# dotnetpower/infomesh

Hardware: AMD Instinct MI355X
Metric: queries/sec (hybrid BM25+dense search, 1.25M docs) (higher is better)
Workload: dtype bf16; 1 GPU; model=bge-small-en(random-init) encoder + BM25 CSR + cosine top-k, global_batch=128, seq_len=32, parallelism=shard1, mode=hybrid, docs_per_gpu=1250000, total_docs=1250000

## Files before the change

### infomesh_amd/models/bert.py

```python
from __future__ import annotations

from dataclasses import dataclass

import torch

from ..ops import kernels as K
from ..ops import reference as R


@dataclass(frozen=True)
class BertConfig:
    vocab_size: int
    hidden: int
    layers: int
    heads: int
    ffn: int
    max_pos: int = 512
    eps: float = 1e-12

    @property
    def head_dim(self) -> int:
        return self.hidden // self.heads


# ... 32 lines not shown
        t = v.to(device)
        out[k] = t if k.endswith(".b") and "ln" not in k else t.to(dtype)
        if "ln" in k:
            out[k] = t.to(dtype)
    return out


class BertEncoder:
    def __init__(self, cfg: BertConfig, weights: dict[str, torch.Tensor],
                 use_fused_attn: bool = True):
        self.cfg = cfg
        self.w = weights
        self.use_fused_attn = use_fused_attn and cfg.head_dim in (32, 64,
                                                                  96, 128)

    def forward(self, ids: torch.Tensor, lens: torch.Tensor) -> torch.Tensor:
        cfg, w = self.cfg, self.w
        B, S = ids.shape
        if S % 32 != 0:
            pad = 32 - S % 32
            ids = torch.nn.functional.pad(ids, (0, pad))
            S += pad
        H, nh, d = cfg.hidden, cfg.heads, cfg.head_dim
        pos_ids = torch.arange(S, device=ids.device, dtype=torch.int32)\
            .repeat(B)
        x = K.gather(w["embed.word"], ids.reshape(-1))
        x = K.add(x, K.gather(w["embed.pos"], pos_ids))
        x = K.layernorm(x, w["embed.ln.g"], w["embed.ln.b"], eps=cfg.eps)

        vl = lens.repeat_interleave(nh).contiguous()
        scale = d ** -0.5
        vl_b = lens.contiguous()
        for i in range(cfg.layers):
            p = f"layer.{i}."
            qkv = K.gemm_nt(x, w[p + "qkv.w"], bias=w[p + "qkv.b"])
            if self.use_fused_attn:
                qkv5 = qkv.view(B, S, 3, nh, d)
                qv = qkv5[:, :, 0].permute(0, 2, 1, 3)
                kv = qkv5[:, :, 1].permute(0, 2, 1, 3)
                vv = qkv5[:, :, 2].permute(0, 2, 1, 3)
                ctx = K.attn_fused(qv, kv, vv, valid_len=vl_b, scale=scale)
            else:
                q, k, vt = K.qkv_split(qkv, B, S, nh, nh, d)
                scores = K.gemm_nt(q, k, out_f32=True, alpha=scale)
                probs = K.softmax(scores, valid_len=vl)
                ctx = K.gemm_nt(probs, vt)
            merged = K.merge_heads(ctx, B, S, nh, d)
            attn = K.gemm_nt(merged, w[p + "attn_out.w"],
                             bias=w[p + "attn_out.b"])
            x = K.layernorm(attn, w[p + "ln1.g"], w[p + "ln1.b"],
                            residual=x, eps=cfg.eps)
            h = K.gemm_nt(x, w[p + "ffn_in.w"], bias=w[p + "ffn_in.b"],
                          act="gelu")
            o = K.gemm_nt(h, w[p + "ffn_out.w"], bias=w[p + "ffn_out.b"])
            x = K.layernorm(o, w[p + "ln2.g"], w[p + "ln2.b"],
                            residual=x, eps=cfg.eps)
        return x.view(B, S, H)

    def forward_reference(self, ids: torch.Tensor,
                          lens: torch.Tensor) -> torch.Tensor:
        cfg = self.cfg
        w = {k: v.float().cpu() for k, v in self.w.items()}
        B, S = ids.shape
        H, nh, d = cfg.hidden, cfg.heads, cfg.head_dim
        ids_l = ids.cpu().long()
        x = w["embed.word"][ids_l] + w["embed.pos"][:S].unsqueeze(0)
        x = R.layernorm(x, w["embed.ln.g"], w["embed.ln.b"], eps=cfg.eps)
        vl = lens.cpu().repeat_interleave(nh)
        for i in range(cfg.layers):
            p = f"layer.{i}."
            qkv = R.gemm_nt(x.view(B * S, H), w[p + "qkv.w"], w[p + "qkv.b"])
            qkv = qkv.view(B, S, 3, nh, d)
# ... 16 lines not shown
```

### infomesh_amd/models/encoder.py

```python
from __future__ import annotations

import torch

from ..ops import kernels as K
from ..ops import reference as R
from .bert import BertConfig, BertEncoder, init_bert_weights
from .tokenizer import HashTokenizer

BGE_SMALL = BertConfig(vocab_size=30522, hidden=384, layers=12, heads=12,
                       ffn=1536, max_pos=512)

EMBED_DIM = BGE_SMALL.hidden


class EmbeddingEncoder:

    def __init__(self, device: str = "cuda", seed: int = 1234,
                 cfg: BertConfig = BGE_SMALL, max_len: int = 128,
                 use_graph: bool = True):
        self.cfg = cfg
        self.device = device
        self.max_len = max_len
        self.tokenizer = HashTokenizer(cfg.vocab_size)
        self.bert = BertEncoder(cfg, init_bert_weights(cfg, seed, device))
        from ..ops.graphs import GraphedCallable
        self._graphed = GraphedCallable(self._encode_impl, enabled=use_graph)

    def _encode_impl(self, ids: torch.Tensor,
                     lens: torch.Tensor) -> torch.Tensor:
        hidden = self.bert.forward(ids, lens)
        return K.pool(hidden, lens, mode="cls", l2=True)

    def encode_ids(self, ids: torch.Tensor, lens: torch.Tensor) -> torch.Tensor:
        return self._graphed(ids, lens)

    def encode_texts(self, texts: list[str]) -> torch.Tensor:
        ids_l, lens = self.tokenizer.encode_batch(texts, self.max_len)
        ids = torch.tensor(ids_l, dtype=torch.int32, device=self.device)
        lens_t = torch.tensor(lens, dtype=torch.int32, device=self.device)
        return self.encode_ids(ids, lens_t)

    def encode_ids_reference(self, ids: torch.Tensor,
                             lens: torch.Tensor) -> torch.Tensor:
        hidden = self.bert.forward_reference(ids, lens)
        return R.pool(hidden.bfloat16(), lens.cpu(), mode="cls", l2=True)
```

### infomesh_amd/models/phi3.py

```python
from __future__ import annotations

from dataclasses import dataclass

import torch

from ..ops import kernels as K
from ..ops import reference as R


@dataclass(frozen=True)
class Phi3Config:
    vocab_size: int = 32064
    hidden: int = 3072
    layers: int = 32
    heads: int = 32
    kv_heads: int = 32
    ffn: int = 8192
    max_pos: int = 4096
    rope_theta: float = 10000.0
    eps: float = 1e-5

    @property
    def head_dim(self) -> int:
        return self.hidden // self.heads
# ... 82 lines not shown
        x = K.gather(self.w["embed"], ids.reshape(-1))
        scale = d ** -0.5
        fused = d in (32, 64, 96, 128)
        for i in range(cfg.layers):
            p = f"layer.{i}."
            h = K.rmsnorm(x, self.w[p + "ln1.g"], eps=cfg.eps)
            qkv = K.gemm_nt(h, self.w[p + "qkv.w"])
            qh, kh, vt = K.qkv_split(qkv, B, S, nh, nkv, d,
                                     cos_t=self.cos, sin_t=self.sin,
                                     pos=pos, want_vt=not fused)
            v_view = qkv.view(B, S, nh + 2 * nkv, d)[:, :, nh + nkv:]\
                .permute(0, 2, 1, 3)
            self.k_cache[i][:B, :, :S] = kh.view(B, nkv, S, d)
            self.v_cache[i][:B, :, :S] = v_view
            if fused:
                ctx = K.attn_fused(qh.view(B, nh, S, d),
                                   kh.view(B, nkv, S, d), v_view,
                                   causal=True, scale=scale)
            else:
                if nh != nkv:
                    rep = nh // nkv
                    kh = kh.view(B, nkv, 1, S, d)\
                        .expand(B, nkv, rep, S, d)\
                        .reshape(B * nh, S, d).contiguous()
                    vt = vt.view(B, nkv, 1, d, S)\
                        .expand(B, nkv, rep, d, S)\
                        .reshape(B * nh, d, S).contiguous()
                scores = K.gemm_nt(qh, kh, out_f32=True, alpha=scale)
                probs = K.softmax(scores, causal=True)
                ctx = K.gemm_nt(probs, vt)
            merged = K.merge_heads(ctx, B, S, nh, d)
            attn = K.gemm_nt(merged, self.w[p + "o.w"])
            x = K.add(x, attn)
            h2 = K.rmsnorm(x, self.w[p + "ln2.g"], eps=cfg.eps)
            gu = K.gemm_nt(h2, self.w[p + "gate_up.w"])
            mlp = K.gemm_nt(K.silu_mul_fused(gu, cfg.ffn),
                            self.w[p + "down.w"])
            x = K.add(x, mlp)
        self.lens[:B] = S_true
        self._len_host = max(self._len_host, S_true)
        x_last = x.view(B, S, H)[:, S_true - 1, :].contiguous()
        h = K.rmsnorm(x_last, self.w["final_ln.g"], eps=cfg.eps)
        return K.gemm_nt(h, self.w["lm_head"], out_f32=True)

    def decode_step(self, ids: torch.Tensor) -> torch.Tensor:
        B = ids.shape[0]
# ... 119 lines not shown
```

### infomesh_amd/models/reranker.py

```python
from __future__ import annotations

import torch

from ..ops import kernels as K
from .bert import BertConfig, BertEncoder, init_bert_weights
from .tokenizer import HashTokenizer, PAD

BGE_RERANKER_BASE = BertConfig(vocab_size=250002, hidden=768, layers=12,
                               heads=12, ffn=3072, max_pos=512)


class CrossEncoderReranker:
    def __init__(self, device: str = "cuda", seed: int = 4321,
                 cfg: BertConfig = BGE_RERANKER_BASE, max_len: int = 160,
                 batch: int = 256):
        self.cfg = cfg
        self.device = device
        self.max_len = max_len
        self.batch = batch
        self.tokenizer = HashTokenizer(cfg.vocab_size)
        self.bert = BertEncoder(cfg, init_bert_weights(cfg, seed, device))
        g = torch.Generator().manual_seed(seed + 1)
        self.cls_w = (torch.randn(1, cfg.hidden, generator=g) * 0.02)\
            .to(device).bfloat16()
        self.cls_b = torch.zeros(1, device=device)

    def score_ids(self, ids: torch.Tensor, lens: torch.Tensor) -> torch.Tensor:
        hidden = self.bert.forward(ids, lens)
        cls = K.pool(hidden, lens, mode="cls", l2=False)
        logits = K.gemm_nt(cls.bfloat16(), self.cls_w, bias=self.cls_b,
                           out_f32=True)
        return logits.view(-1)

    def score_pairs(self, query: str, passages: list[str]) -> torch.Tensor:
        out = []
        for i in range(0, len(passages), self.batch):
            chunk = passages[i:i + self.batch]
            enc = [self.tokenizer.encode_pair(query, p, self.max_len)
                   for p in chunk]
            lens = [len(e) for e in enc]
            width = max(lens)
            ids = torch.tensor([e + [PAD] * (width - len(e)) for e in enc],
                               dtype=torch.int32, device=self.device)
            lens_t = torch.tensor(lens, dtype=torch.int32, device=self.device)
# ... 11 lines not shown
```

### infomesh_amd/ops/_ext.py

```python
from __future__ import annotations

import ctypes
from ctypes import c_float, c_int, c_long, c_void_p
from pathlib import Path

from ..errors import GpuExtensionMissing

_LIB: ctypes.CDLL | None = None
_LOAD_ERROR: str | None = None

_SIGNATURES: dict[str, list] = {
    "infomesh_gemm_bf16_nt": [c_void_p, c_void_p, c_void_p, c_void_p,
                              c_int, c_int, c_int, c_int,
                              c_long, c_long, c_long,
                              c_int, c_float, c_int, c_void_p],
    "infomesh_layernorm": [c_void_p, c_void_p, c_void_p, c_void_p,
                           c_void_p, c_void_p, c_long, c_int, c_float,
                           c_void_p],
    "infomesh_rmsnorm": [c_void_p, c_void_p, c_void_p, c_void_p,
                         c_void_p, c_long, c_int, c_float, c_void_p],
    "infomesh_softmax": [c_void_p, c_void_p, c_void_p, c_long, c_int,
                         c_int, c_int, c_float, c_void_p],
    "infomesh_bias_act": [c_void_p, c_void_p, c_long, c_int, c_int, c_void_p],
    "infomesh_silu_mul": [c_void_p, c_void_p, c_void_p, c_long, c_void_p],
# ... 24 lines not shown
    "infomesh_simhash_fingerprint": [c_void_p, c_void_p, c_void_p, c_long,
                                     c_void_p],
    "infomesh_hamming_scan": [c_void_p, c_void_p, c_void_p, c_void_p,
                              c_void_p, c_void_p, c_int, c_long, c_int,
                              c_int, c_void_p],
    "infomesh_attn_decode": [c_void_p, c_void_p, c_void_p, c_void_p,
                             c_void_p, c_int, c_int, c_int, c_int, c_int,
                             c_float, c_void_p],
    "infomesh_attn_decode_split": [c_void_p, c_void_p, c_void_p, c_void_p,
                                   c_void_p, c_void_p, c_int, c_int, c_int,
                                   c_int, c_int, c_int, c_float, c_void_p],
    "infomesh_attn_fused": [c_void_p, c_void_p, c_void_p, c_void_p,
                            c_void_p, c_int, c_int, c_int, c_int, c_int,
                            c_int, c_long, c_long, c_long, c_long, c_long,
                            c_long, c_long, c_long, c_long,
                            c_int, c_float, c_void_p],
    "infomesh_kv_append": [c_void_p, c_void_p, c_void_p, c_void_p,
                           c_void_p, c_int, c_int, c_int, c_int, c_void_p],
    "infomesh_dense_scores": [c_void_p, c_void_p, c_void_p,
                              c_int, c_long, c_int, c_float, c_void_p],
    "infomesh_dense_scores_fp8": [c_void_p, c_void_p, c_void_p,
                                  c_int, c_long, c_int, c_float,
                                  c_void_p],
    "infomesh_gemm8_bf16_nt": [c_void_p, c_void_p, c_void_p, c_void_p,
                               c_int, c_int, c_int, c_int,
                               c_long, c_long, c_long,
                               c_int, c_float, c_int, c_void_p],
    "infomesh_gemv_bf16_nt": [c_void_p, c_void_p, c_void_p, c_void_p,
                              c_int, c_int, c_int, c_int,
                              c_long, c_long, c_long,
                              c_int, c_float, c_int, c_void_p],
# ... 96 lines not shown
```

### infomesh_amd/ops/csrc/attn_fused.hip

```cpp
#include "common.h"

#define QTILE 64
#define KTILE 64
#define VPAD 72

struct TensorView {
  const bf16* ptr;
  long bs, hs, rs;
};

namespace {

template <int D>
__global__ __launch_bounds__(256) void attn_fused_kernel(
    TensorView Q, TensorView K, TensorView V,
    const int* __restrict__ valid_len,
    bf16* __restrict__ O, int nhq, int nhk,
    int Sq, int Sk, int causal, float scale) {
  __shared__ bf16 k_lds[KTILE][D];
  __shared__ bf16 vt_lds[D][VPAD];
  __shared__ bf16 p_lds[4][16][KTILE];
  const int g = blockIdx.y;
  const int q0 = blockIdx.x * QTILE;
  const int lane = threadIdx.x & 63;
  const int wid = threadIdx.x >> 6;
  const int b = g / nhq, hq = g % nhq;
  const int hk = hq / (nhq / nhk);
  const int limit_all = valid_len ? min(Sk, valid_len[b]) : Sk;

  const bf16* Qg = Q.ptr + (long)b * Q.bs + (long)hq * Q.hs;
  const bf16* Kg = K.ptr + (long)b * K.bs + (long)hk * K.hs;
  const bf16* Vg = V.ptr + (long)b * V.bs + (long)hk * V.hs;

  const int qrow_f = lane & 15;
  const int kslice = lane >> 4;
  bf16x8 qfrag[D / 32];
  {
    const int qr = min(q0 + wid * 16 + qrow_f, Sq - 1);
// ... 2 lines not shown
      qfrag[f] = *reinterpret_cast<const bf16x8*>(
          Qg + (long)qr * Q.rs + f * 32 + kslice * 8);
  }

  f32x4 o_acc[D / 16];
#pragma unroll
  for (int f = 0; f < D / 16; ++f) o_acc[f] = f32x4{0.f, 0.f, 0.f, 0.f};
  float m_run[4], l_run[4];
#pragma unroll
  for (int r = 0; r < 4; ++r) { m_run[r] = -INFINITY; l_run[r] = 0.f; }
  const int crow0 = (lane >> 4) * 4;
  const int ccol = lane & 15;

  int kv_limit = limit_all;
  if (causal) {
    const int max_q = min(q0 + QTILE - 1, Sq - 1);
    kv_limit = min(kv_limit, max_q + (Sk - Sq) + 1);
  }

  for (int kv0 = 0; kv0 < kv_limit; kv0 += KTILE) {
    {
      const int perrow = D / 8;
      for (int t = threadIdx.x; t < KTILE * perrow; t += 256) {
        const int key = t / perrow, dc = (t % perrow) * 8;
        const int src = min(kv0 + key, Sk - 1);
        *reinterpret_cast<bf16x8*>(&k_lds[key][dc]) =
            *reinterpret_cast<const bf16x8*>(Kg + (long)src * K.rs + dc);
        const bf16x8 vv = *reinterpret_cast<const bf16x8*>(
            Vg + (long)src * V.rs + dc);
#pragma unroll
        for (int j = 0; j < 8; ++j) vt_lds[dc + j][key] = vv[j];
      }
    }
    __syncthreads();

    f32x4 s_chunk[KTILE / 16];
#pragma unroll
    for (int kc = 0; kc < KTILE / 16; ++kc) {
      f32x4 acc = f32x4{0.f, 0.f, 0.f, 0.f};
#pragma unroll
      for (int f = 0; f < D / 32; ++f) {
        const bf16x8 kf = *reinterpret_cast<const bf16x8*>(
            &k_lds[kc * 16 + qrow_f][f * 32 + kslice * 8]);
        acc = __builtin_amdgcn_mfma_f32_16x16x32_bf16(
            qfrag[f], kf, acc, 0, 0, 0);
      }
      s_chunk[kc] = acc;
    }

    float tile_max[4];
#pragma unroll
    for (int r = 0; r < 4; ++r) tile_max[r] = -INFINITY;
#pragma unroll
    for (int kc = 0; kc < KTILE / 16; ++kc) {
      const int key = kv0 + kc * 16 + ccol;
      const bool key_ok = key < limit_all;
#pragma unroll
      for (int r = 0; r < 4; ++r) {
        const int qrow = q0 + wid * 16 + crow0 + r;
        bool ok = key_ok && qrow < Sq;
        if (causal) ok = ok && key <= qrow + (Sk - Sq);
        float v = ok ? s_chunk[kc][r] * scale : -INFINITY;
        s_chunk[kc][r] = v;
        tile_max[r] = fmaxf(tile_max[r], v);
      }
    }
#pragma unroll
    for (int r = 0; r < 4; ++r) {
#pragma unroll
      for (int off = 1; off < 16; off <<= 1)
        tile_max[r] = fmaxf(tile_max[r],
                            __shfl_xor(tile_max[r], off, 64));
    }

    float alpha[4];
#pragma unroll
    for (int r = 0; r < 4; ++r) {
      const float m_new = fmaxf(m_run[r], tile_max[r]);
      alpha[r] = (m_run[r] > -INFINITY) ? __expf(m_run[r] - m_new) : 0.f;
      m_run[r] = m_new;
    }
    float row_sum[4] = {0.f, 0.f, 0.f, 0.f};
#pragma unroll
    for (int kc = 0; kc < KTILE / 16; ++kc) {
#pragma unroll
      for (int r = 0; r < 4; ++r) {
        const float p = (s_chunk[kc][r] > -INFINITY && m_run[r] > -INFINITY)
            ? __expf(s_chunk[kc][r] - m_run[r]) : 0.f;
        s_chunk[kc][r] = p;
        row_sum[r] += p;
      }
    }
#pragma unroll
    for (int r = 0; r < 4; ++r) {
#pragma unroll
      for (int off = 1; off < 16; off <<= 1)
        row_sum[r] += __shfl_xor(row_sum[r], off, 64);
      l_run[r] = l_run[r] * alpha[r] + row_sum[r];
    }

#pragma unroll
    for (int f = 0; f < D / 16; ++f)
#pragma unroll
      for (int r = 0; r < 4; ++r) o_acc[f][r] *= alpha[r];

#pragma unroll
    for (int kc = 0; kc < KTILE / 16; ++kc)
#pragma unroll
      for (int r = 0; r < 4; ++r)
        p_lds[wid][crow0 + r][kc * 16 + ccol] = f2bf(s_chunk[kc][r]);

#pragma unroll
    for (int f = 0; f < D / 16; ++f) {
#pragma unroll
      for (int ks = 0; ks < KTILE / 32; ++ks) {
        const bf16x8 pf = *reinterpret_cast<const bf16x8*>(
            &p_lds[wid][qrow_f][ks * 32 + kslice * 8]);
        const bf16x8 vf = *reinterpret_cast<const bf16x8*>(
            &vt_lds[f * 16 + qrow_f][ks * 32 + kslice * 8]);
        o_acc[f] = __builtin_amdgcn_mfma_f32_16x16x32_bf16(
            pf, vf, o_acc[f], 0, 0, 0);
      }
    }
    __syncthreads();
  }

#pragma unroll
  for (int f = 0; f < D / 16; ++f) {
#pragma unroll
    for (int r = 0; r < 4; ++r) {
      const int qrow = q0 + wid * 16 + crow0 + r;
      if (qrow >= Sq) continue;
      const float inv = l_run[r] > 0.f ? 1.0f / l_run[r] : 0.f;
      O[(long)g * Sq * D + (long)qrow * D + f * 16 + ccol] =
          f2bf(o_acc[f][r] * inv);
    }
  }
}

}

extern "C" void infomesh_attn_fused(
    const void* Q, const void* K, const void* V, const void* valid_len,
    void* O, int B, int nhq, int nhk, int Sq, int Sk, int D,
    long qb, long qh, long qr, long kb, long kh, long kr,
    long vb, long vh, long vr,
    int causal, float scale, void* stream) {
  auto s = reinterpret_cast<hipStream_t>(stream);
  dim3 grid((Sq + QTILE - 1) / QTILE, B * nhq), block(256);
  TensorView qv{(const bf16*)Q, qb, qh, qr};
  TensorView kv{(const bf16*)K, kb, kh, kr};
  TensorView vv{(const bf16*)V, vb, vh, vr};
#define CASE(DV)                                                          \
  case DV:                                                                \
    hipLaunchKernelGGL(attn_fused_kernel<DV>, grid, block, 0, s,          \
                       qv, kv, vv, (const int*)valid_len, (bf16*)O,       \
                       nhq, nhk, Sq, Sk, causal, scale);                  \
    break;
  switch (D) {
    CASE(32) CASE(64) CASE(96) CASE(128)
    default:
      break;
  }
#undef CASE
}
```

### infomesh_amd/ops/csrc/norms.hip

```cpp
#include "common.h"

namespace {

template <bool RMS, bool RESIDUAL>
__global__ __launch_bounds__(256) void norm_kernel(
    const bf16* __restrict__ x, const bf16* __restrict__ res,
    bf16* __restrict__ out, bf16* __restrict__ res_out,
    const bf16* __restrict__ gamma, const bf16* __restrict__ beta,
    int H, float eps) {
  __shared__ float scratch[16];
  const long row = blockIdx.x;
  const bf16* xr = x + row * H;
  const bf16* rr = RESIDUAL ? res + row * H : nullptr;

  constexpr int MAXV = 8;
  f32x4 keep[2 * MAXV];
  const int nvec = H / 8;
  float sum = 0.f, sumsq = 0.f;
  for (int v = threadIdx.x, it = 0; v < nvec; v += blockDim.x, ++it) {
    bf16x8 xv = *reinterpret_cast<const bf16x8*>(xr + v * 8);
    float f[8];
#pragma unroll
    for (int j = 0; j < 8; ++j) f[j] = bf2f(xv[j]);
    if (RESIDUAL) {
      bf16x8 rv = *reinterpret_cast<const bf16x8*>(rr + v * 8);
#pragma unroll
      for (int j = 0; j < 8; ++j) f[j] += bf2f(rv[j]);
      if (res_out) {
// ... 39 lines not shown
    bf16x8 ov;
    if (!RMS && beta) {
      bf16x8 bv = *reinterpret_cast<const bf16x8*>(beta + v * 8);
#pragma unroll
      for (int j = 0; j < 8; ++j)
        ov[j] = f2bf((f[j] - mean) * inv * bf2f(gv[j]) + bf2f(bv[j]));
    } else {
#pragma unroll
      for (int j = 0; j < 8; ++j)
        ov[j] = f2bf((f[j] - (RMS ? 0.f : mean)) * inv * bf2f(gv[j]));
    }
    *reinterpret_cast<bf16x8*>(out + row * H + v * 8) = ov;
  }
}

template <bool RMS, bool RESIDUAL>
__global__ __launch_bounds__(256) void norm_rowwave_kernel(
    const bf16* __restrict__ x, const bf16* __restrict__ res,
    bf16* __restrict__ out, bf16* __restrict__ res_out,
    const bf16* __restrict__ gamma, const bf16* __restrict__ beta,
    long rows, int H, float eps) {
  const long row = (long)blockIdx.x * 4 + (threadIdx.x >> 6);
  if (row >= rows) return;
  const int lane = threadIdx.x & 63;
  const bf16* xr = x + row * H;
  const bf16* rr = RESIDUAL ? res + row * H : nullptr;
  const int nvec = H / 8;
  float f[8 * 4];
  float sum = 0.f, sumsq = 0.f;
  int it = 0;
  for (int v = lane; v < nvec; v += 64, ++it) {
    bf16x8 xv = *reinterpret_cast<const bf16x8*>(xr + v * 8);
#pragma unroll
    for (int j = 0; j < 8; ++j) f[it * 8 + j] = bf2f(xv[j]);
    if (RESIDUAL) {
      bf16x8 rv = *reinterpret_cast<const bf16x8*>(rr + v * 8);
#pragma unroll
      for (int j = 0; j < 8; ++j) f[it * 8 + j] += bf2f(rv[j]);
      if (res_out) {
        bf16x8 ov;
#pragma unroll
        for (int j = 0; j < 8; ++j) ov[j] = f2bf(f[it * 8 + j]);
        *reinterpret_cast<bf16x8*>(res_out + row * H + v * 8) = ov;
      }
    }
#pragma unroll
    for (int j = 0; j < 8; ++j) {
      sum += f[it * 8 + j];
      sumsq += f[it * 8 + j] * f[it * 8 + j];
    }
  }
  float mean = 0.f;
  if (!RMS) mean = wave_reduce_sum(sum) / H;
  const float ms = wave_reduce_sum(sumsq) / H;
  const float inv = rsqrtf((RMS ? ms : ms - mean * mean) + eps);
  it = 0;
  for (int v = lane; v < nvec; v += 64, ++it) {
    bf16x8 gv = *reinterpret_cast<const bf16x8*>(gamma + v * 8);
    bf16x8 ov;
    if (!RMS && beta) {
      bf16x8 bv = *reinterpret_cast<const bf16x8*>(beta + v * 8);
#pragma unroll
      for (int j = 0; j < 8; ++j)
        ov[j] = f2bf((f[it * 8 + j] - mean) * inv * bf2f(gv[j])
                     + bf2f(bv[j]));
    } else {
#pragma unroll
      for (int j = 0; j < 8; ++j)
        ov[j] = f2bf((f[it * 8 + j] - (RMS ? 0.f : mean)) * inv
                     * bf2f(gv[j]));
    }
    *reinterpret_cast<bf16x8*>(out + row * H + v * 8) = ov;
  }
}

}

#define NORM_LAUNCH(RMS, RES, ...)                                        \
  do {                                                                    \
    if (H <= 2048) {                                                      \
      dim3 g((unsigned)((rows + 3) / 4));                                 \
      hipLaunchKernelGGL((norm_rowwave_kernel<RMS, RES>), g, dim3(256),   \
                         0, s, __VA_ARGS__, rows, H, eps);                \
    } else {                                                              \
      dim3 g((unsigned)rows);                                             \
      hipLaunchKernelGGL((norm_kernel<RMS, RES>), g, dim3(256), 0, s,     \
                         __VA_ARGS__, H, eps);                            \
    }                                                                     \
  } while (0)

extern "C" void infomesh_layernorm(
    const void* x, const void* residual, void* out, void* res_out,
    const void* gamma, const void* beta,
    long rows, int H, float eps, void* stream) {
  auto s = reinterpret_cast<hipStream_t>(stream);
  if (residual)
    NORM_LAUNCH(false, true, (const bf16*)x, (const bf16*)residual,
                (bf16*)out, (bf16*)res_out, (const bf16*)gamma,
                (const bf16*)beta);
  else
    NORM_LAUNCH(false, false, (const bf16*)x, nullptr, (bf16*)out,
                nullptr, (const bf16*)gamma, (const bf16*)beta);
}

extern "C" void infomesh_rmsnorm(
    const void* x, const void* residual, void* out, void* res_out,
    const void* gamma, long rows, int H, float eps, void* stream) {
  auto s = reinterpret_cast<hipStream_t>(stream);
  if (residual)
    NORM_LAUNCH(true, true, (const bf16*)x, (const bf16*)residual,
                (bf16*)out, (bf16*)res_out, (const bf16*)gamma, nullptr);
  else
    NORM_LAUNCH(true, false, (const bf16*)x, nullptr, (bf16*)out,
                nullptr, (const bf16*)gamma, nullptr);
}
```

### infomesh_amd/ops/kernels.py

```python
from __future__ import annotations

import torch

from . import _ext

ACT = {"none": 0, "gelu": 1, "silu": 2, "relu": 3, "tanh": 4}


def _ptr(t: torch.Tensor | None) -> int | None:
    return None if t is None else t.data_ptr()


def _check(t: torch.Tensor, dtype: torch.dtype, name: str) -> None:
    assert t.is_cuda, f"{name} must be on GPU"
    assert t.dtype == dtype, f"{name} must be {dtype}, got {t.dtype}"
    assert t.is_contiguous(), f"{name} must be contiguous"


def gemm_route(M: int, N: int, K: int, G: int) -> str:
    if M <= 16:
        return "gemv"
    if (M >= 4096 and N >= 512 and K % 64 == 0
            and ((M + 255) // 256) * ((N + 255) // 256) * max(G, 1) >= 224):
        return "gemm8"
# ... 2 lines not shown

_GEMM_ENTRY = {"gemv": "infomesh_gemv_bf16_nt",
               "gemm8": "infomesh_gemm8_bf16_nt",
               "gemm": "infomesh_gemm_bf16_nt"}


def gemm_tile(M: int, N: int, K: int, G: int) -> tuple[int, int, int, bool]:
    code = _ext.lib().infomesh_gemm_tile(M, N, K, G)
    return code & 0xff, code >> 8 & 0xff, code >> 16 & 0xff, bool(code >> 24)


def gemm_nt(a: torch.Tensor, b: torch.Tensor,
            bias: torch.Tensor | None = None,
            act: str = "none", alpha: float = 1.0,
            out_f32: bool = False,
            out: torch.Tensor | None = None) -> torch.Tensor:
    sq_a = a.dim() == 2
    if sq_a:
        a = a.unsqueeze(0)
    if b.dim() == 2:
        b = b.unsqueeze(0).expand(a.shape[0], *b.shape)
    G, M, K = a.shape
    Gb, N, Kb = b.shape
    assert K == Kb and Gb == G, f"shape mismatch {a.shape} x {b.shape}"
    assert K % 32 == 0, f"K={K} must be a multiple of 32"
    _check(a, torch.bfloat16, "A")
    assert b.dtype == torch.bfloat16
    strideB = 0 if (G > 1 and b.stride(0) == 0) else N * K
    if strideB != 0:
        assert b.is_contiguous()
    else:
        assert b[0].is_contiguous()
    if bias is not None:
        _check(bias, torch.float32, "bias")
        assert bias.numel() == N
    dtype = torch.float32 if out_f32 else torch.bfloat16
    if out is None:
        out = torch.empty((G, M, N), device=a.device, dtype=dtype)
    else:
        assert out.shape == (G, M, N) and out.dtype == dtype and out.is_contiguous()
    fn = getattr(_ext.lib(), _GEMM_ENTRY[gemm_route(M, N, K, G)])
    fn(a.data_ptr(), b.data_ptr(), out.data_ptr(), _ptr(bias),
       M, N, K, G, M * K, strideB, M * N,
       ACT[act], alpha, int(out_f32), _ext.stream_ptr())
    return out.squeeze(0) if sq_a else out


def gemm_bmax_width(M: int, N: int, K: int, G: int = 1) -> int:
    if gemm_route(M, N, K, G) != "gemm":
        return 0
    return _ext.lib().infomesh_gemm_bmax_width(M, N, K, G)


def gemm_nt_bmax(a: torch.Tensor, b: torch.Tensor, alpha: float = 1.0,
                 out: torch.Tensor | None = None,
                 bmax: torch.Tensor | None = None
# ... 49 lines not shown
    rc = _ext.lib().infomesh_dense_scores_fp8(
        a.data_ptr(), b.data_ptr(), out.data_ptr(), M, N, K, alpha,
        _ext.stream_ptr())
    return out if rc == 0 else None


def layernorm(x: torch.Tensor, gamma: torch.Tensor, beta: torch.Tensor,
              residual: torch.Tensor | None = None, eps: float = 1e-12,
              return_residual: bool = False):
    H = x.shape[-1]
    assert H % 8 == 0
    rows = x.numel() // H
    _check(x, torch.bfloat16, "x")
    out = torch.empty_like(x)
    res_out = None
    if residual is not None:
        assert residual.shape == x.shape
        if return_residual:
            res_out = torch.empty_like(x)
    _ext.lib().infomesh_layernorm(
        x.data_ptr(), _ptr(residual), out.data_ptr(), _ptr(res_out),
        gamma.data_ptr(), beta.data_ptr(), rows, H, eps, _ext.stream_ptr())
    return (out, res_out) if return_residual else out


def rmsnorm(x: torch.Tensor, gamma: torch.Tensor,
            residual: torch.Tensor | None = None, eps: float = 1e-5,
            return_residual: bool = False):
    H = x.shape[-1]
    assert H % 8 == 0
    rows = x.numel() // H
    _check(x, torch.bfloat16, "x")
    out = torch.empty_like(x)
    res_out = None
    if residual is not None and return_residual:
        res_out = torch.empty_like(x)
    _ext.lib().infomesh_rmsnorm(
        x.data_ptr(), _ptr(residual), out.data_ptr(), _ptr(res_out),
# ... 242 lines not shown
                 ) -> tuple[torch.Tensor, torch.Tensor, torch.Tensor]:
    M, N = queries.numel(), table.numel()
    dev = table.device
    out_q = torch.empty(cap, device=dev, dtype=torch.int32)
    out_n = torch.empty(cap, device=dev, dtype=torch.int32)
    out_d = torch.empty(cap, device=dev, dtype=torch.int32)
    cnt = torch.zeros(1, device=dev, dtype=torch.int32)
    _ext.lib().infomesh_hamming_scan(
        queries.data_ptr(), table.data_ptr(), out_q.data_ptr(),
        out_n.data_ptr(), out_d.data_ptr(), cnt.data_ptr(), M, N, radius,
        cap, _ext.stream_ptr())
    n = min(int(cnt.item()), cap)
    return out_q[:n], out_n[:n], out_d[:n]


def attn_fused(q: torch.Tensor, k: torch.Tensor, v: torch.Tensor,
               valid_len: torch.Tensor | None = None,
               causal: bool = False, scale: float | None = None
               ) -> torch.Tensor:
    assert q.dim() == 4 and k.dim() == 4 and v.dim() == 4
    B, nh, Sq, d = q.shape
    _, nhk, Sk, dk = k.shape
    assert d == dk and d in (32, 64, 96, 128) and nh % nhk == 0
    for t in (q, k, v):
        assert t.dtype == torch.bfloat16 and t.stride(3) == 1
    if scale is None:
        scale = d ** -0.5
    out = torch.empty(B * nh, Sq, d, device=q.device, dtype=torch.bfloat16)
    if valid_len is not None:
        _check(valid_len, torch.int32, "valid_len")
        assert valid_len.numel() == B
    _ext.lib().infomesh_attn_fused(
        q.data_ptr(), k.data_ptr(), v.data_ptr(), _ptr(valid_len),
        out.data_ptr(), B, nh, nhk, Sq, Sk, d,
        q.stride(0), q.stride(1), q.stride(2),
        k.stride(0), k.stride(1), k.stride(2),
        v.stride(0), v.stride(1), v.stride(2),
        int(causal), scale, _ext.stream_ptr())
    return out


def attn_decode(q: torch.Tensor, k_cache: torch.Tensor,
                v_cache: torch.Tensor, lens: torch.Tensor,
                scale: float) -> torch.Tensor:
    import math
    B, H, D = q.shape
    _, Hkv, Smax, _ = k_cache.shape
    _check(q, torch.bfloat16, "q")
    assert D % 8 == 0 and D <= 128
    out = torch.empty_like(q)
    nc_min = max(1, math.ceil(Smax / 2048))
    nc = max(nc_min, min(64, math.ceil(512 / max(1, B * H))))
    if nc <= 1:
# ... 62 lines not shown
```

Measured before the change: 44210 queries/s.

## Compute only CLS row in last BERT layer, fuse embed+LN, short-seq attention variants

Restricts the final encoder layer to the CLS token: its attention, output projection, FFN and layernorm run on one row per sequence instead of all S rows. Adds a fused embedding-gather+add+layernorm kernel and has attention write its output directly in merged-head layout, which removes the separate merge_heads pass. Also adds specialised short-sequence attention variants with smaller key tiles and fewer waves when Sq and Sk are at most 32. The CLS tail is only taken when the GEMM router would choose the plain GEMM path, so numerics match the full-sequence path; the cost is more code paths and strided-residual support in layernorm.

```diff
diff --git a/infomesh_amd/models/bert.py b/infomesh_amd/models/bert.py
--- a/infomesh_amd/models/bert.py
+++ b/infomesh_amd/models/bert.py
@@ -70,48 +70,96 @@
         self.use_fused_attn = use_fused_attn and cfg.head_dim in (32, 64,
                                                                   96, 128)
 
+    @staticmethod
+    def _pad_ids(ids: torch.Tensor) -> torch.Tensor:
+        S = ids.shape[1]
+        if S % 32 != 0:
+            ids = torch.nn.functional.pad(ids, (0, 32 - S % 32))
+        return ids
+
+    def _embed(self, ids: torch.Tensor) -> torch.Tensor:
+        cfg, w = self.cfg, self.w
+        return K.embed_layernorm(w["embed.word"], w["embed.pos"],
+                                 ids.reshape(-1), ids.shape[1],
+                                 w["embed.ln.g"], w["embed.ln.b"],
+                                 eps=cfg.eps)
+
+    def _layer(self, i: int, x: torch.Tensor, B: int, S: int,
+               lens: torch.Tensor) -> torch.Tensor:
+        cfg, w = self.cfg, self.w
+        nh, d = cfg.heads, cfg.head_dim
+        scale = d ** -0.5
+        p = f"layer.{i}."
+        qkv = K.gemm_nt(x, w[p + "qkv.w"], bias=w[p + "qkv.b"])
+        if self.use_fused_attn:
+            qkv5 = qkv.view(B, S, 3, nh, d)
+            qv = qkv5[:, :, 0].permute(0, 2, 1, 3)
+            kv = qkv5[:, :, 1].permute(0, 2, 1, 3)
+            vv = qkv5[:, :, 2].permute(0, 2, 1, 3)
+            merged = K.attn_fused(qv, kv, vv, valid_len=lens, scale=scale,
+                                  out_merged=True)
+        else:
+            vl = lens.repeat_interleave(nh).contiguous()
+            q, k, vt = K.qkv_split(qkv, B, S, nh, nh, d)
+            scores = K.gemm_nt(q, k, out_f32=True, alpha=scale)
+            probs = K.softmax(scores, valid_len=vl)
+            ctx = K.gemm_nt(probs, vt)
+            merged = K.merge_heads(ctx, B, S, nh, d)
+        attn = K.gemm_nt(merged, w[p + "attn_out.w"],
+                         bias=w[p + "attn_out.b"])
+        x = K.layernorm(attn, w[p + "ln1.g"], w[p + "ln1.b"],
+                        residual=x, eps=cfg.eps)
+        h = K.gemm_nt(x, w[p + "ffn_in.w"], bias=w[p + "ffn_in.b"],
+                      act="gelu")
+        o = K.gemm_nt(h, w[p + "ffn_out.w"], bias=w[p + "ffn_out.b"])
+        return K.layernorm(o, w[p + "ln2.g"], w[p + "ln2.b"],
+                           residual=x, eps=cfg.eps)
+
     def forward(self, ids: torch.Tensor, lens: torch.Tensor) -> torch.Tensor:
+        ids = self._pad_ids(ids)
+        B, S = ids.shape
+        x = self._embed(ids)
+        lens = lens.contiguous()
+        for i in range(self.cfg.layers):
+            x = self._layer(i, x, B, S, lens)
+        return x.view(B, S, self.cfg.hidden)
+
+    def cls_tail_exact(self, B: int, S: int) -> bool:
+        H, F = self.cfg.hidden, self.cfg.ffn
+        return self.use_fused_attn and all(
+            K.gemm_route(B * S, N, Kd, 1) == "gemm"
+            for N, Kd in ((H, H), (F, H), (H, F)))
+
+    def forward_cls(self, ids: torch.Tensor,
+                    lens: torch.Tensor) -> torch.Tensor:
+        ids = self._pad_ids(ids)
+        B, S = ids.shape
+        if not self.cls_tail_exact(B, S):
+            return self.forward(ids, lens)[:, 0].contiguous()
         cfg, w = self.cfg, self.w
-        B, S = ids.shape
-        if S % 32 != 0:
-            pad = 32 - S % 32
-            ids = torch.nn.functional.pad(ids, (0, pad))
-            S += pad
         H, nh, d = cfg.hidden, cfg.heads, cfg.head_dim
-        pos_ids = torch.arange(S, device=ids.device, dtype=torch.int32)\
-            .repeat(B)
-        x = K.gather(w["embed.word"], ids.reshape(-1))
-        x = K.add(x, K.gather(w["embed.pos"], pos_ids))
-        x = K.layernorm(x, w["embed.ln.g"], w["embed.ln.b"], eps=cfg.eps)
-
-        vl = lens.repeat_interleave(nh).contiguous()
-        scale = d ** -0.5
-        vl_b = lens.contiguous()
-        for i in range(cfg.layers):
-            p = f"layer.{i}."
-            qkv = K.gemm_nt(x, w[p + "qkv.w"], bias=w[p + "qkv.b"])
-            if self.use_fused_attn:
-                qkv5 = qkv.view(B, S, 3, nh, d)
-                qv = qkv5[:, :, 0].permute(0, 2, 1, 3)
-                kv = qkv5[:, :, 1].permute(0, 2, 1, 3)
-                vv = qkv5[:, :, 2].permute(0, 2, 1, 3)
-                ctx = K.attn_fused(qv, kv, vv, valid_len=vl_b, scale=scale)
-            else:
-                q, k, vt = K.qkv_split(qkv, B, S, nh, nh, d)
-                scores = K.gemm_nt(q, k, out_f32=True, alpha=scale)
-                probs = K.softmax(scores, valid_len=vl)
-                ctx = K.gemm_nt(probs, vt)
-            merged = K.merge_heads(ctx, B, S, nh, d)
-            attn = K.gemm_nt(merged, w[p + "attn_out.w"],
-                             bias=w[p + "attn_out.b"])
-            x = K.layernorm(attn, w[p + "ln1.g"], w[p + "ln1.b"],
-                            residual=x, eps=cfg.eps)
-            h = K.gemm_nt(x, w[p + "ffn_in.w"], bias=w[p + "ffn_in.b"],
-                          act="gelu")
-            o = K.gemm_nt(h, w[p + "ffn_out.w"], bias=w[p + "ffn_out.b"])
-            x = K.layernorm(o, w[p + "ln2.g"], w[p + "ln2.b"],
-                            residual=x, eps=cfg.eps)
-        return x.view(B, S, H)
+        x = self._embed(ids)
+        lens = lens.contiguous()
+        for i in range(cfg.layers - 1):
+            x = self._layer(i, x, B, S, lens)
+        p = f"layer.{cfg.layers - 1}."
+        qkv5 = K.gemm_nt(x, w[p + "qkv.w"], bias=w[p + "qkv.b"])\
+            .view(B, S, 3, nh, d)
+        merged = K.attn_fused(qkv5[:, 0:1, 0].permute(0, 2, 1, 3),
+                              qkv5[:, :, 1].permute(0, 2, 1, 3),
+                              qkv5[:, :, 2].permute(0, 2, 1, 3),
+                              valid_len=lens, scale=d ** -0.5,
+                              out_merged=True)
+        attn = K.gemm_nt(merged, w[p + "attn_out.w"],
+                         bias=w[p + "attn_out.b"], route="gemm")
+        x = K.layernorm(attn, w[p + "ln1.g"], w[p + "ln1.b"],
+                        residual=x.view(B, S, H)[:, 0], eps=cfg.eps)
+        h = K.gemm_nt(x, w[p + "ffn_in.w"], bias=w[p + "ffn_in.b"],
+                      act="gelu", route="gemm")
+        o = K.gemm_nt(h, w[p + "ffn_out.w"], bias=w[p + "ffn_out.b"],
+                      route="gemm")
+        return K.layernorm(o, w[p + "ln2.g"], w[p + "ln2.b"],
+                           residual=x, eps=cfg.eps)
 
     def forward_reference(self, ids: torch.Tensor,
                           lens: torch.Tensor) -> torch.Tensor:
diff --git a/infomesh_amd/models/encoder.py b/infomesh_amd/models/encoder.py
--- a/infomesh_amd/models/encoder.py
+++ b/infomesh_amd/models/encoder.py
@@ -28,8 +28,8 @@
 
     def _encode_impl(self, ids: torch.Tensor,
                      lens: torch.Tensor) -> torch.Tensor:
-        hidden = self.bert.forward(ids, lens)
-        return K.pool(hidden, lens, mode="cls", l2=True)
+        cls = self.bert.forward_cls(ids, lens)
+        return K.pool(cls.unsqueeze(1), lens, mode="cls", l2=True)
 
     def encode_ids(self, ids: torch.Tensor, lens: torch.Tensor) -> torch.Tensor:
         return self._graphed(ids, lens)
diff --git a/infomesh_amd/models/phi3.py b/infomesh_amd/models/phi3.py
--- a/infomesh_amd/models/phi3.py
+++ b/infomesh_amd/models/phi3.py
@@ -120,9 +120,10 @@
             self.k_cache[i][:B, :, :S] = kh.view(B, nkv, S, d)
             self.v_cache[i][:B, :, :S] = v_view
             if fused:
-                ctx = K.attn_fused(qh.view(B, nh, S, d),
-                                   kh.view(B, nkv, S, d), v_view,
-                                   causal=True, scale=scale)
+                merged = K.attn_fused(qh.view(B, nh, S, d),
+                                      kh.view(B, nkv, S, d), v_view,
+                                      causal=True, scale=scale,
+                                      out_merged=True)
             else:
                 if nh != nkv:
                     rep = nh // nkv
@@ -135,7 +136,7 @@
                 scores = K.gemm_nt(qh, kh, out_f32=True, alpha=scale)
                 probs = K.softmax(scores, causal=True)
                 ctx = K.gemm_nt(probs, vt)
-            merged = K.merge_heads(ctx, B, S, nh, d)
+                merged = K.merge_heads(ctx, B, S, nh, d)
             attn = K.gemm_nt(merged, self.w[p + "o.w"])
             x = K.add(x, attn)
             h2 = K.rmsnorm(x, self.w[p + "ln2.g"], eps=cfg.eps)
diff --git a/infomesh_amd/models/reranker.py b/infomesh_amd/models/reranker.py
--- a/infomesh_amd/models/reranker.py
+++ b/infomesh_amd/models/reranker.py
@@ -26,8 +26,9 @@
         self.cls_b = torch.zeros(1, device=device)
 
     def score_ids(self, ids: torch.Tensor, lens: torch.Tensor) -> torch.Tensor:
-        hidden = self.bert.forward(ids, lens)
-        cls = K.pool(hidden, lens, mode="cls", l2=False)
+        hidden = self.bert.forward_cls(ids, lens)
+        cls = K.pool(hidden.unsqueeze(1), lens, mode="cls",
+                     l2=False)
         logits = K.gemm_nt(cls.bfloat16(), self.cls_w, bias=self.cls_b,
                            out_f32=True)
         return logits.view(-1)
diff --git a/infomesh_amd/ops/_ext.py b/infomesh_amd/ops/_ext.py
--- a/infomesh_amd/ops/_ext.py
+++ b/infomesh_amd/ops/_ext.py
@@ -62,7 +62,14 @@
                             c_void_p, c_int, c_int, c_int, c_int, c_int,
                             c_int, c_long, c_long, c_long, c_long, c_long,
                             c_long, c_long, c_long, c_long,
-                            c_int, c_float, c_void_p],
+                            c_long, c_long, c_long,
+                            c_int, c_float, c_int, c_void_p],
+    "infomesh_layernorm_rs": [c_void_p, c_void_p, c_long, c_void_p,
+                              c_void_p, c_void_p, c_void_p, c_long, c_int,
+                              c_float, c_void_p],
+    "infomesh_embed_layernorm": [c_void_p, c_void_p, c_void_p, c_void_p,
+                                 c_void_p, c_void_p, c_long, c_int, c_int,
+                                 c_float, c_void_p],
     "infomesh_kv_append": [c_void_p, c_void_p, c_void_p, c_void_p,
                            c_void_p, c_int, c_int, c_int, c_int, c_void_p],
     "infomesh_dense_scores": [c_void_p, c_void_p, c_void_p,
diff --git a/infomesh_amd/ops/csrc/attn_fused.hip b/infomesh_amd/ops/csrc/attn_fused.hip
--- a/infomesh_amd/ops/csrc/attn_fused.hip
+++ b/infomesh_amd/ops/csrc/attn_fused.hip
@@ -1,27 +1,32 @@
 #include "common.h"
 
-#define QTILE 64
 #define KTILE 64
-#define VPAD 72
+#define KTILE_SHORT 32
 
 struct TensorView {
   const bf16* ptr;
   long bs, hs, rs;
 };
+struct OutView {
+  bf16* ptr;
+  long bs, hs, rs;
+};
 
 namespace {
 
-template <int D>
-__global__ __launch_bounds__(256) void attn_fused_kernel(
+template <int D, int KT, int NW>
+__global__ __launch_bounds__(NW * 64) void attn_fused_kernel(
     TensorView Q, TensorView K, TensorView V,
     const int* __restrict__ valid_len,
-    bf16* __restrict__ O, int nhq, int nhk,
+    OutView O, int nhq, int nhk,
     int Sq, int Sk, int causal, float scale) {
-  __shared__ bf16 k_lds[KTILE][D];
+  constexpr int QT = NW * 16;
+  constexpr int VPAD = KT + 8;
+  __shared__ bf16 k_lds[KT][D];
   __shared__ bf16 vt_lds[D][VPAD];
-  __shared__ bf16 p_lds[4][16][KTILE];
+  __shared__ bf16 p_lds[NW][16][KT];
   const int g = blockIdx.y;
-  const int q0 = blockIdx.x * QTILE;
+  const int q0 = blockIdx.x * QT;
   const int lane = threadIdx.x & 63;
   const int wid = threadIdx.x >> 6;
   const int b = g / nhq, hq = g % nhq;
@@ -54,14 +59,14 @@
 
   int kv_limit = limit_all;
   if (causal) {
-    const int max_q = min(q0 + QTILE - 1, Sq - 1);
+    const int max_q = min(q0 + QT - 1, Sq - 1);
     kv_limit = min(kv_limit, max_q + (Sk - Sq) + 1);
   }
 
-  for (int kv0 = 0; kv0 < kv_limit; kv0 += KTILE) {
+  for (int kv0 = 0; kv0 < kv_limit; kv0 += KT) {
     {
       const int perrow = D / 8;
-      for (int t = threadIdx.x; t < KTILE * perrow; t += 256) {
+      for (int t = threadIdx.x; t < KT * perrow; t += NW * 64) {
         const int key = t / perrow, dc = (t % perrow) * 8;
         const int src = min(kv0 + key, Sk - 1);
         *reinterpret_cast<bf16x8*>(&k_lds[key][dc]) =
@@ -74,9 +79,9 @@
     }
     __syncthreads();
 
-    f32x4 s_chunk[KTILE / 16];
-#pragma unroll
-    for (int kc = 0; kc < KTILE / 16; ++kc) {
+    f32x4 s_chunk[KT / 16];
+#pragma unroll
+    for (int kc = 0; kc < KT / 16; ++kc) {
       f32x4 acc = f32x4{0.f, 0.f, 0.f, 0.f};
 #pragma unroll
       for (int f = 0; f < D / 32; ++f) {
@@ -92,7 +97,7 @@
 #pragma unroll
     for (int r = 0; r < 4; ++r) tile_max[r] = -INFINITY;
 #pragma unroll
-    for (int kc = 0; kc < KTILE / 16; ++kc) {
+    for (int kc = 0; kc < KT / 16; ++kc) {
       const int key = kv0 + kc * 16 + ccol;
       const bool key_ok = key < limit_all;
 #pragma unroll
@@ -122,7 +127,7 @@
     }
     float row_sum[4] = {0.f, 0.f, 0.f, 0.f};
 #pragma unroll
-    for (int kc = 0; kc < KTILE / 16; ++kc) {
+    for (int kc = 0; kc < KT / 16; ++kc) {
 #pragma unroll
       for (int r = 0; r < 4; ++r) {
         const float p = (s_chunk[kc][r] > -INFINITY && m_run[r] > -INFINITY)
@@ -145,7 +150,7 @@
       for (int r = 0; r < 4; ++r) o_acc[f][r] *= alpha[r];
 
 #pragma unroll
-    for (int kc = 0; kc < KTILE / 16; ++kc)
+    for (int kc = 0; kc < KT / 16; ++kc)
 #pragma unroll
       for (int r = 0; r < 4; ++r)
         p_lds[wid][crow0 + r][kc * 16 + ccol] = f2bf(s_chunk[kc][r]);
@@ -153,7 +158,7 @@
 #pragma unroll
     for (int f = 0; f < D / 16; ++f) {
 #pragma unroll
-      for (int ks = 0; ks < KTILE / 32; ++ks) {
+      for (int ks = 0; ks < KT / 32; ++ks) {
         const bf16x8 pf = *reinterpret_cast<const bf16x8*>(
             &p_lds[wid][qrow_f][ks * 32 + kslice * 8]);
         const bf16x8 vf = *reinterpret_cast<const bf16x8*>(
@@ -165,6 +170,7 @@
     __syncthreads();
   }
 
+  bf16* Og = O.ptr + (long)b * O.bs + (long)hq * O.hs;
 #pragma unroll
   for (int f = 0; f < D / 16; ++f) {
 #pragma unroll
@@ -172,10 +178,18 @@
       const int qrow = q0 + wid * 16 + crow0 + r;
       if (qrow >= Sq) continue;
       const float inv = l_run[r] > 0.f ? 1.0f / l_run[r] : 0.f;
-      O[(long)g * Sq * D + (long)qrow * D + f * 16 + ccol] =
-          f2bf(o_acc[f][r] * inv);
-    }
-  }
+      Og[(long)qrow * O.rs + f * 16 + ccol] = f2bf(o_acc[f][r] * inv);
+    }
+  }
+}
+
+template <int D, int KT, int NW>
+void launch(hipStream_t s, TensorView q, TensorView k, TensorView v,
+            const int* valid_len, OutView o, int B, int nhq, int nhk,
+            int Sq, int Sk, int causal, float scale) {
+  dim3 grid((Sq + NW * 16 - 1) / (NW * 16), B * nhq), block(NW * 64);
+  hipLaunchKernelGGL((attn_fused_kernel<D, KT, NW>), grid, block, 0, s,
+                     q, k, v, valid_len, o, nhq, nhk, Sq, Sk, causal, scale);
 }
 
 }
@@ -184,23 +198,32 @@
     const void* Q, const void* K, const void* V, const void* valid_len,
     void* O, int B, int nhq, int nhk, int Sq, int Sk, int D,
     long qb, long qh, long qr, long kb, long kh, long kr,
-    long vb, long vh, long vr,
-    int causal, float scale, void* stream) {
+    long vb, long vh, long vr, long ob, long oh, long orow,
+    int causal, float scale, int variant, void* stream) {
   auto s = reinterpret_cast<hipStream_t>(stream);
-  dim3 grid((Sq + QTILE - 1) / QTILE, B * nhq), block(256);
   TensorView qv{(const bf16*)Q, qb, qh, qr};
   TensorView kv{(const bf16*)K, kb, kh, kr};
   TensorView vv{(const bf16*)V, vb, vh, vr};
-#define CASE(DV)                                                          \
-  case DV:                                                                \
-    hipLaunchKernelGGL(attn_fused_kernel<DV>, grid, block, 0, s,          \
-                       qv, kv, vv, (const int*)valid_len, (bf16*)O,       \
-                       nhq, nhk, Sq, Sk, causal, scale);                  \
-    break;
+  OutView ov{(bf16*)O, ob, oh, orow};
+  const int* vl = (const int*)valid_len;
+#define ARGS s, qv, kv, vv, vl, ov, B, nhq, nhk, Sq, Sk, causal, scale
+  if (variant != 0 && (D == 32 || D == 64)) {
+    if (D == 32) {
+      if (variant == 1) launch<32, KTILE_SHORT, 2>(ARGS);
+      else launch<32, KTILE_SHORT, 1>(ARGS);
+    } else {
+      if (variant == 1) launch<64, KTILE_SHORT, 2>(ARGS);
+      else launch<64, KTILE_SHORT, 1>(ARGS);
+    }
+    return;
+  }
   switch (D) {
-    CASE(32) CASE(64) CASE(96) CASE(128)
+    case 32: launch<32, KTILE, 4>(ARGS); break;
+    case 64: launch<64, KTILE, 4>(ARGS); break;
+    case 96: launch<96, KTILE, 4>(ARGS); break;
+    case 128: launch<128, KTILE, 4>(ARGS); break;
     default:
       break;
   }
-#undef CASE
-}
+#undef ARGS
+}
diff --git a/infomesh_amd/ops/csrc/norms.hip b/infomesh_amd/ops/csrc/norms.hip
--- a/infomesh_amd/ops/csrc/norms.hip
+++ b/infomesh_amd/ops/csrc/norms.hip
@@ -7,11 +7,11 @@
     const bf16* __restrict__ x, const bf16* __restrict__ res,
     bf16* __restrict__ out, bf16* __restrict__ res_out,
     const bf16* __restrict__ gamma, const bf16* __restrict__ beta,
-    int H, float eps) {
+    int H, float eps, long res_rs) {
   __shared__ float scratch[16];
   const long row = blockIdx.x;
   const bf16* xr = x + row * H;
-  const bf16* rr = RESIDUAL ? res + row * H : nullptr;
+  const bf16* rr = RESIDUAL ? res + row * res_rs : nullptr;
 
   constexpr int MAXV = 8;
   f32x4 keep[2 * MAXV];
@@ -81,17 +81,56 @@
   }
 }
 
+__device__ __forceinline__ void rowwave_accum(const float* f8, float& sum,
+                                              float& sumsq) {
+#pragma unroll
+  for (int j = 0; j < 8; ++j) {
+    sum += f8[j];
+    sumsq += f8[j] * f8[j];
+  }
+}
+
+template <bool RMS>
+__device__ __forceinline__ void rowwave_finish(
+    const float* f, float sum, float sumsq, int lane, int H, float eps,
+    const bf16* __restrict__ gamma, const bf16* __restrict__ beta,
+    bf16* __restrict__ out_row) {
+  const int nvec = H / 8;
+  float mean = 0.f;
+  if (!RMS) mean = wave_reduce_sum(sum) / H;
+  const float ms = wave_reduce_sum(sumsq) / H;
+  const float inv = rsqrtf((RMS ? ms : ms - mean * mean) + eps);
+  int it = 0;
+  for (int v = lane; v < nvec; v += 64, ++it) {
+    bf16x8 gv = *reinterpret_cast<const bf16x8*>(gamma + v * 8);
+    bf16x8 ov;
+    if (!RMS && beta) {
+      bf16x8 bv = *reinterpret_cast<const bf16x8*>(beta + v * 8);
+#pragma unroll
+      for (int j = 0; j < 8; ++j)
+        ov[j] = f2bf((f[it * 8 + j] - mean) * inv * bf2f(gv[j])
+                     + bf2f(bv[j]));
+    } else {
+#pragma unroll
+      for (int j = 0; j < 8; ++j)
+        ov[j] = f2bf((f[it * 8 + j] - (RMS ? 0.f : mean)) * inv
+                     * bf2f(gv[j]));
+    }
+    *reinterpret_cast<bf16x8*>(out_row + v * 8) = ov;
+  }
+}
+
 template <bool RMS, bool RESIDUAL>
 __global__ __launch_bounds__(256) void norm_rowwave_kernel(
     const bf16* __restrict__ x, const bf16* __restrict__ res,
     bf16* __restrict__ out, bf16* __restrict__ res_out,
     const bf16* __restrict__ gamma, const bf16* __restrict__ beta,
-    long rows, int H, float eps) {
+    long rows, int H, float eps, long res_rs) {
   const long row = (long)blockIdx.x * 4 + (threadIdx.x >> 6);
   if (row >= rows) return;
   const int lane = threadIdx.x & 63;
   const bf16* xr = x + row * H;
-  const bf16* rr = RESIDUAL ? res + row * H : nullptr;
+  const bf16* rr = RESIDUAL ? res + row * res_rs : nullptr;
   const int nvec = H / 8;
   float f[8 * 4];
   float sum = 0.f, sumsq = 0.f;
@@ -111,34 +150,36 @@
         *reinterpret_cast<bf16x8*>(res_out + row * H + v * 8) = ov;
       }
     }
-#pragma unroll
-    for (int j = 0; j < 8; ++j) {
-      sum += f[it * 8 + j];
-      sumsq += f[it * 8 + j] * f[it * 8 + j];
-    }
-  }
-  float mean = 0.f;
-  if (!RMS) mean = wave_reduce_sum(sum) / H;
-  const float ms = wave_reduce_sum(sumsq) / H;
-  const float inv = rsqrtf((RMS ? ms : ms - mean * mean) + eps);
-  it = 0;
+    rowwave_accum(f + it * 8, sum, sumsq);
+  }
+  rowwave_finish<RMS>(f, sum, sumsq, lane, H, eps, gamma, beta,
+                      out + row * H);
+}
+
+__global__ __launch_bounds__(256) void embed_layernorm_kernel(
+    const bf16* __restrict__ word, const bf16* __restrict__ pos,
+    const int* __restrict__ ids, bf16* __restrict__ out,
+    const bf16* __restrict__ gamma, const bf16* __restrict__ beta,
+    long rows, int S, int H, float eps) {
+  const long row = (long)blockIdx.x * 4 + (threadIdx.x >> 6);
+  if (row >= rows) return;
+  const int lane = threadIdx.x & 63;
+  const bf16* wr = word + (long)ids[row] * H;
+  const bf16* pr = pos + (row % S) * H;
+  const int nvec = H / 8;
+  float f[8 * 4];
+  float sum = 0.f, sumsq = 0.f;
+  int it = 0;
   for (int v = lane; v < nvec; v += 64, ++it) {
-    bf16x8 gv = *reinterpret_cast<const bf16x8*>(gamma + v * 8);
-    bf16x8 ov;
-    if (!RMS && beta) {
-      bf16x8 bv = *reinterpret_cast<const bf16x8*>(beta + v * 8);
-#pragma unroll
-      for (int j = 0; j < 8; ++j)
-        ov[j] = f2bf((f[it * 8 + j] - mean) * inv * bf2f(gv[j])
-                     + bf2f(bv[j]));
-    } else {
-#pragma unroll
-      for (int j = 0; j < 8; ++j)
-        ov[j] = f2bf((f[it * 8 + j] - (RMS ? 0.f : mean)) * inv
-                     * bf2f(gv[j]));
-    }
-    *reinterpret_cast<bf16x8*>(out + row * H + v * 8) = ov;
-  }
+    bf16x8 wv = *reinterpret_cast<const bf16x8*>(wr + v * 8);
+    bf16x8 pv = *reinterpret_cast<const bf16x8*>(pr + v * 8);
+#pragma unroll
+    for (int j = 0; j < 8; ++j)
+      f[it * 8 + j] = bf2f(f2bf(bf2f(wv[j]) + bf2f(pv[j])));
+    rowwave_accum(f + it * 8, sum, sumsq);
+  }
+  rowwave_finish<false>(f, sum, sumsq, lane, H, eps, gamma, beta,
+                        out + row * H);
 }
 
 }
@@ -148,17 +189,17 @@
     if (H <= 2048) {                                                      \
       dim3 g((unsigned)((rows + 3) / 4));                                 \
       hipLaunchKernelGGL((norm_rowwave_kernel<RMS, RES>), g, dim3(256),   \
-                         0, s, __VA_ARGS__, rows, H, eps);                \
+                         0, s, __VA_ARGS__, rows, H, eps, res_rs);        \
     } else {                                                              \
       dim3 g((unsigned)rows);                                             \
       hipLaunchKernelGGL((norm_kernel<RMS, RES>), g, dim3(256), 0, s,     \
-                         __VA_ARGS__, H, eps);                            \
+                         __VA_ARGS__, H, eps, res_rs);                    \
     }                                                                     \
   } while (0)
 
-extern "C" void infomesh_layernorm(
-    const void* x, const void* residual, void* out, void* res_out,
-    const void* gamma, const void* beta,
+extern "C" void infomesh_layernorm_rs(
+    const void* x, const void* residual, long res_rs, void* out,
+    void* res_out, const void* gamma, const void* beta,
     long rows, int H, float eps, void* stream) {
   auto s = reinterpret_cast<hipStream_t>(stream);
   if (residual)
@@ -170,9 +211,36 @@
                 nullptr, (const bf16*)gamma, (const bf16*)beta);
 }
 
+extern "C" void infomesh_embed_layernorm(
+    const void* word, const void* pos, const void* ids, void* out,
+    const void* gamma, const void* beta, long rows, int S, int H,
+    float eps, void* stream) {
+  auto s = reinterpret_cast<hipStream_t>(stream);
+  hipLaunchKernelGGL(embed_layernorm_kernel, dim3((unsigned)((rows + 3) / 4)),
+                     dim3(256), 0, s, (const bf16*)word, (const bf16*)pos,
+                     (const int*)ids, (bf16*)out, (const bf16*)gamma,
+                     (const bf16*)beta, rows, S, H, eps);
+}
+
+extern "C" void infomesh_layernorm(
+    const void* x, const void* residual, void* out, void* res_out,
+    const void* gamma, const void* beta,
+    long rows, int H, float eps, void* stream) {
+  const long res_rs = H;
+  auto s = reinterpret_cast<hipStream_t>(stream);
+  if (residual)
+    NORM_LAUNCH(false, true, (const bf16*)x, (const bf16*)residual,
+                (bf16*)out, (bf16*)res_out, (const bf16*)gamma,
+                (const bf16*)beta);
+  else
+    NORM_LAUNCH(false, false, (const bf16*)x, nullptr, (bf16*)out,
+                nullptr, (const bf16*)gamma, (const bf16*)beta);
+}
+
 extern "C" void infomesh_rmsnorm(
     const void* x, const void* residual, void* out, void* res_out,
     const void* gamma, long rows, int H, float eps, void* stream) {
+  const long res_rs = H;
   auto s = reinterpret_cast<hipStream_t>(stream);
   if (residual)
     NORM_LAUNCH(true, true, (const bf16*)x, (const bf16*)residual,
diff --git a/infomesh_amd/ops/kernels.py b/infomesh_amd/ops/kernels.py
--- a/infomesh_amd/ops/kernels.py
+++ b/infomesh_amd/ops/kernels.py
@@ -40,7 +40,8 @@
             bias: torch.Tensor | None = None,
             act: str = "none", alpha: float = 1.0,
             out_f32: bool = False,
-            out: torch.Tensor | None = None) -> torch.Tensor:
+            out: torch.Tensor | None = None,
+            route: str | None = None) -> torch.Tensor:
     sq_a = a.dim() == 2
     if sq_a:
         a = a.unsqueeze(0)
@@ -65,7 +66,9 @@
         out = torch.empty((G, M, N), device=a.device, dtype=dtype)
     else:
         assert out.shape == (G, M, N) and out.dtype == dtype and out.is_contiguous()
-    fn = getattr(_ext.lib(), _GEMM_ENTRY[gemm_route(M, N, K, G)])
+    assert route in (None, "gemm"), f"cannot force route {route!r}"
+    fn = getattr(_ext.lib(),
+                 _GEMM_ENTRY[route or gemm_route(M, N, K, G)])
     fn(a.data_ptr(), b.data_ptr(), out.data_ptr(), _ptr(bias),
        M, N, K, G, M * K, strideB, M * N,
        ACT[act], alpha, int(out_f32), _ext.stream_ptr())
@@ -145,14 +148,39 @@
     _check(x, torch.bfloat16, "x")
     out = torch.empty_like(x)
     res_out = None
+    res_rs = H
     if residual is not None:
         assert residual.shape == x.shape
+        assert residual.dtype == torch.bfloat16
+        if not residual.is_contiguous():
+            assert residual.dim() == 2 and residual.stride(1) == 1, \
+                "strided residual must be [rows, H] with unit column stride"
+            res_rs = residual.stride(0)
         if return_residual:
             res_out = torch.empty_like(x)
-    _ext.lib().infomesh_layernorm(
-        x.data_ptr(), _ptr(residual), out.data_ptr(), _ptr(res_out),
-        gamma.data_ptr(), beta.data_ptr(), rows, H, eps, _ext.stream_ptr())
+    _ext.lib().infomesh_layernorm_rs(
+        x.data_ptr(), _ptr(residual), res_rs, out.data_ptr(),
+        _ptr(res_out), gamma.data_ptr(), beta.data_ptr(), rows, H, eps,
+        _ext.stream_ptr())
     return (out, res_out) if return_residual else out
+
+
+def embed_layernorm(word: torch.Tensor, pos: torch.Tensor,
+                    ids: torch.Tensor, S: int, gamma: torch.Tensor,
+                    beta: torch.Tensor, eps: float = 1e-12) -> torch.Tensor:
+    _check(word, torch.bfloat16, "word")
+    _check(pos, torch.bfloat16, "pos")
+    _check(ids, torch.int32, "ids")
+    H = word.shape[1]
+    assert pos.shape[1] == H and H % 8 == 0 and H <= 2048
+    assert 1 <= S <= pos.shape[0] and ids.numel() % S == 0
+    out = torch.empty((ids.numel(), H), device=word.device,
+                      dtype=torch.bfloat16)
+    _ext.lib().infomesh_embed_layernorm(
+        word.data_ptr(), pos.data_ptr(), ids.data_ptr(), out.data_ptr(),
+        gamma.data_ptr(), beta.data_ptr(), ids.numel(), S, H, eps,
+        _ext.stream_ptr())
+    return out
 
 
 def rmsnorm(x: torch.Tensor, gamma: torch.Tensor,
@@ -425,9 +453,19 @@
     return out_q[:n], out_n[:n], out_d[:n]
 
 
+_ATTN_VARIANT = {"generic": 0, "short32": 1, "short16": 2}
+
+
+def attn_variant(Sq: int, Sk: int, d: int) -> str:
+    if Sq <= 32 and Sk <= 32 and d in (32, 64):
+        return "short16" if Sq <= 16 else "short32"
+    return "generic"
+
+
 def attn_fused(q: torch.Tensor, k: torch.Tensor, v: torch.Tensor,
                valid_len: torch.Tensor | None = None,
-               causal: bool = False, scale: float | None = None
+               causal: bool = False, scale: float | None = None,
+               out_merged: bool = False, variant: str | None = None
                ) -> torch.Tensor:
     assert q.dim() == 4 and k.dim() == 4 and v.dim() == 4
     B, nh, Sq, d = q.shape
@@ -437,7 +475,16 @@
         assert t.dtype == torch.bfloat16 and t.stride(3) == 1
     if scale is None:
         scale = d ** -0.5
-    out = torch.empty(B * nh, Sq, d, device=q.device, dtype=torch.bfloat16)
+    assert variant in (None, "generic"), f"cannot force variant {variant!r}"
+    code = _ATTN_VARIANT[variant or attn_variant(Sq, Sk, d)]
+    if out_merged:
+        out = torch.empty(B * Sq, nh * d, device=q.device,
+                          dtype=torch.bfloat16)
+        ob, oh, orow = Sq * nh * d, d, nh * d
+    else:
+        out = torch.empty(B * nh, Sq, d, device=q.device,
+                          dtype=torch.bfloat16)
+        ob, oh, orow = nh * Sq * d, Sq * d, d
     if valid_len is not None:
         _check(valid_len, torch.int32, "valid_len")
         assert valid_len.numel() == B
@@ -447,7 +494,7 @@
         q.stride(0), q.stride(1), q.stride(2),
         k.stride(0), k.stride(1), k.stride(2),
         v.stride(0), v.stride(1), v.stride(2),
-        int(causal), scale, _ext.stream_ptr())
+        ob, oh, orow, int(causal), scale, code, _ext.stream_ptr())
     return out
 
 
```

New measurement: 44560 queries/s, median of 4. No clear change (+0.8%).
